# stone-d-chen/ffvvc

Measured on AMD Instinct MI355X. Metric: decoded frames/sec (4K/8K 10-bit VVC) per GPU, higher is better.
Workload: dtype u16

## Files before the change

### ffvvc_amd/csrc/loopfilter.hip

```cpp
#include "common.hpp"
#include "runtime.hpp"
#include "bs_rules.hpp"
#include "../../include/vvc_mi355.h"
#include "stage_checks.hpp"

namespace vvc355 {


template <int BD>
__global__ __launch_bounds__(256) void lmcs_kernel(const vvc355_blend_job *__restrict__ jobs)
{
    using px_t = typename Px<BD>::type;
    constexpr int VB = 8 * (int)sizeof(px_t);
    __shared__ __attribute__((aligned(16))) px_t lut_lds[1 << BD];
    const vvc355_blend_job job = load_uniform(jobs + (blockIdx.y));
    const uint8_t *lut = (const uint8_t *)job.src0;
    if ((job.src0 & 15) == 0) {
        for (int i = threadIdx.x; i < (int)((sizeof(px_t) << BD) / 16); i += 256)
            ((uint4 *)lut_lds)[i] = gld<uint4>(lut + i * 16);
    } else {
        for (int i = threadIdx.x; i < (1 << BD); i += 256)
            lut_lds[i] = (px_t)ld_px<BD>(lut, i);
    }
    __syncthreads();
// ... 430 lines not shown
    __device__ __forceinline__ void vec(int o, int n, int (&e)[4]) const
    {
        const px_t *a = (const px_t *)pix + o;
        if (BD > 8) {
            uint2 v = make_uint2(0, 0);
            if (n == 4) v = gld<uint2>(a); else v.x = gld<uint32_t>(a);
            e[0] = v.x & 0xffff; e[1] = v.x >> 16; e[2] = v.y & 0xffff; e[3] = v.y >> 16;
        } else {
            const uint32_t v = n == 4 ? gld<uint32_t>(a) : (uint32_t)gld<uint16_t>(a);
            e[0] = v & 0xff; e[1] = (v >> 8) & 0xff; e[2] = (v >> 16) & 0xff; e[3] = v >> 24;
        }
    }
    __device__ __forceinline__ void load(int lines, int half, int which)
    {
        const int b = 4 * half;
        if (xs == 1) {
#pragma unroll
            for (int l = 0; l < 4; l++) {
                int e[4];
                if (l < lines && (which & 1)) {
                    vec(l * ys - b - 4, 4, e);
#pragma unroll
                    for (int k = 0; k < 4; k++) P[l][b + 3 - k] = e[k];
                }
                if (l < lines && (which & 2)) {
                    vec(l * ys + b, 4, e);
#pragma unroll
                    for (int k = 0; k < 4; k++) Q[l][b + k] = e[k];
                }
            }
        } else {
#pragma unroll
            for (int i = 0; i < 4; i++) {
                int e[4];
                if (which & 1) {
                    vec(-(b + i + 1) * xs, lines, e);
#pragma unroll
                    for (int l = 0; l < 4; l++) P[l][b + i] = e[l];
                }
                if (which & 2) {
                    vec((b + i) * xs, lines, e);
#pragma unroll
                    for (int l = 0; l < 4; l++) Q[l][b + i] = e[l];
                }
            }
        }
    }
};
__device__ __forceinline__ int d2(int a, int b, int c) { return abs(a - 2 * b + c); }

__device__ __forceinline__ int long_w(int n, int i) { return n == 3 ? 53 - 21 * i : n == 5 ? 58 - 13 * i : 59 - 9 * i; }
__device__ __forceinline__ int long_t(int n, int i) { return n == 3 ? 6 - 2 * i : n == 5 ? 6 - i : max(6 - i, 1); }

template <int BD>
__device__ __forceinline__ void dbk_luma_large(const Dbk<BD> &d, int tc, int no_p, int no_q, int len_p, int len_q)
{
#pragma unroll
    for (int l = 0; l < 4; l++) {
        int p[8], q[8], m;
#pragma unroll
        for (int i = 0; i < 8; i++) { p[i] = d.p(l, i); q[i] = d.q(l, i); }
        if (len_p == 5 && len_q == 5)
            m = (p[4] + p[3] + 2 * (p[2] + p[1] + p[0] + q[0] + q[1] + q[2]) + q[3] + q[4] + 8) >> 4;
        else if (len_p == len_q)
            m = (p[6] + p[5] + p[4] + p[3] + p[2] + p[1] + 2 * (p[0] + q[0]) + q[1] + q[2] + q[3] + q[4] + q[5] + q[6] + 8) >> 4;
        else if (len_p + len_q == 12)
            m = (p[5] + p[4] + p[3] + p[2] + 2 * (p[1] + p[0] + q[0] + q[1]) + q[2] + q[3] + q[4] + q[5] + 8) >> 4;
        else if (len_p + len_q == 8)
            m = (p[3] + p[2] + p[1] + p[0] + q[0] + q[1] + q[2] + q[3] + 4) >> 3;
        else if (len_q == 7)
            m = (2 * (p[2] + p[1] + p[0] + q[0]) + p[0] + p[1] + q[1] + q[2] + q[3] + q[4] + q[5] + q[6] + 8) >> 4;
        else
            m = (p[6] + p[5] + p[4] + p[3] + p[2] + p[1] + 2 * (q[2] + q[1] + q[0] + p[0]) + q[0] + q[1] + 8) >> 4;
        if (!no_p) {
            const int n = len_p == 3 ? 3 : len_p == 5 ? 5 : 7;
            int ref = 0;
#pragma unroll
            for (int i = 0; i < 8; i++) if (i == len_p || i == len_p - 1) ref += p[i];
            ref = (ref + 1) >> 1;
#pragma unroll
            for (int i = 0; i < 7; i++)
                if (i < n) {
                    const int lim = (tc * long_t(n, i)) >> 1, wt = long_w(n, i);
                    d.sp(l, i, p[i] + clip3(((m * wt + ref * (64 - wt) + 32) >> 6) - p[i], -lim, lim));
                }
        }
        if (!no_q) {
            const int n = len_q == 3 ? 3 : len_q == 5 ? 5 : 7;
            int ref = 0;
#pragma unroll
            for (int i = 0; i < 8; i++) if (i == len_q || i == len_q - 1) ref += q[i];
            ref = (ref + 1) >> 1;
#pragma unroll
            for (int i = 0; i < 7; i++)
                if (i < n) {
                    const int lim = (tc * long_t(n, i)) >> 1, wt = long_w(n, i);
                    d.sq(l, i, q[i] + clip3(((m * wt + ref * (64 - wt) + 32) >> 6) - q[i], -lim, lim));
                }
        }
    }
}

template <int BD>
__device__ __forceinline__ void dbk_luma_segment(const Dbk<BD> &d, int tc_in, int beta_in, int no_p, int no_q, int len_p, int len_q, int hor_ctu_edge)
{
    const int tc = BD < 10 ? (tc_in + (1 << (9 - BD))) >> (10 - BD) : tc_in << (BD - 10);
    if (!tc)
        return;
    const int dp0 = d2(d.p(0, 2), d.p(0, 1), d.p(0, 0)), dq0 = d2(d.q(0, 2), d.q(0, 1), d.q(0, 0));
    const int dp3 = d2(d.p(3, 2), d.p(3, 1), d.p(3, 0)), dq3 = d2(d.q(3, 2), d.q(3, 1), d.q(3, 0));
    const int d0 = dp0 + dq0, d3 = dp3 + dq3;
    const int tc25 = (tc * 5 + 1) >> 1;
    const int large_p = len_p > 3 && !hor_ctu_edge, large_q = len_q > 3;
    const int beta = beta_in << (BD - 8);

    if (large_p || large_q) {
        const int dp0l = large_p ? (dp0 + d2(d.p(0, 5), d.p(0, 4), d.p(0, 3)) + 1) >> 1 : dp0;
        const int dq0l = large_q ? (dq0 + d2(d.q(0, 5), d.q(0, 4), d.q(0, 3)) + 1) >> 1 : dq0;
        const int dp3l = large_p ? (dp3 + d2(d.p(3, 5), d.p(3, 4), d.p(3, 3)) + 1) >> 1 : dp3;
        const int dq3l = large_q ? (dq3 + d2(d.q(3, 5), d.q(3, 4), d.q(3, 3)) + 1) >> 1 : dq3;
        const int d0l = dp0l + dq0l, d3l = dp3l + dq3l;
        const int beta53 = (beta * 3) >> 5, beta_4 = beta >> 4;
        len_p = large_p ? len_p : 3;
        len_q = large_q ? len_q : 3;
        if (d0l + d3l < beta) {
            const int sp0l = abs(d.p(0, 3) - d.p(0, 0)) + (len_p == 7 ? abs(d.p(0, 7) - d.p(0, 6) - d.p(0, 5) + d.p(0, 4)) : 0);
            const int sq0l = abs(d.q(0, 0) - d.q(0, 3)) + (len_q == 7 ? abs(d.q(0, 4) - d.q(0, 5) - d.q(0, 6) + d.q(0, 7)) : 0);
            const int sp3l = abs(d.p(3, 3) - d.p(3, 0)) + (len_p == 7 ? abs(d.p(3, 7) - d.p(3, 6) - d.p(3, 5) + d.p(3, 4)) : 0);
            const int sq3l = abs(d.q(3, 0) - d.q(3, 3)) + (len_q == 7 ? abs(d.q(3, 4) - d.q(3, 5) - d.q(3, 6) + d.q(3, 7)) : 0);
            const int sp0 = large_p ? (sp0l + abs(d.p(0, 3) - d.p_at(0, len_p)) + 1) >> 1 : sp0l;
            const int sp3 = large_p ? (sp3l + abs(d.p(3, 3) - d.p_at(3, len_p)) + 1) >> 1 : sp3l;
            const int sq0 = large_q ? (sq0l + abs(d.q(0, 3) - d.q_at(0, len_q)) + 1) >> 1 : sq0l;
            const int sq3 = large_q ? (sq3l + abs(d.q(3, 3) - d.q_at(3, len_q)) + 1) >> 1 : sq3l;
            if (sp0 + sq0 < beta53 && abs(d.p(0, 0) - d.q(0, 0)) < tc25 &&
                sp3 + sq3 < beta53 && abs(d.p(3, 0) - d.q(3, 0)) < tc25 &&
                (d0l << 1) < beta_4 && (d3l << 1) < beta_4) {
                dbk_luma_large<BD>(d, tc, no_p, no_q, len_p, len_q);
                return;
            }
        }
    }
    if (d0 + d3 >= beta)
        return;
    const int beta_3 = beta >> 3, beta_2 = beta >> 2;
    if (len_p > 2 && len_q > 2 &&
        abs(d.p(0, 3) - d.p(0, 0)) + abs(d.q(0, 3) - d.q(0, 0)) < beta_3 && abs(d.p(0, 0) - d.q(0, 0)) < tc25 &&
        abs(d.p(3, 3) - d.p(3, 0)) + abs(d.q(3, 3) - d.q(3, 0)) < beta_3 && abs(d.p(3, 0) - d.q(3, 0)) < tc25 &&
        (d0 << 1) < beta_2 && (d3 << 1) < beta_2) {
        const int tc2 = tc << 1, tc3 = tc * 3;
#pragma unroll
        for (int l = 0; l < 4; l++) {
            const int p3 = d.p(l, 3), p2 = d.p(l, 2), p1 = d.p(l, 1), p0 = d.p(l, 0);
            const int q0 = d.q(l, 0), q1 = d.q(l, 1), q2 = d.q(l, 2), q3 = d.q(l, 3);
            if (!no_p) {
                d.sp(l, 0, p0 + clip3(((p2 + 2 * p1 + 2 * p0 + 2 * q0 + q1 + 4) >> 3) - p0, -tc3, tc3));
                d.sp(l, 1, p1 + clip3(((p2 + p1 + p0 + q0 + 2) >> 2) - p1, -tc2, tc2));
                d.sp(l, 2, p2 + clip3(((2 * p3 + 3 * p2 + p1 + p0 + q0 + 4) >> 3) - p2, -tc, tc));
            }
            if (!no_q) {
                d.sq(l, 0, q0 + clip3(((p1 + 2 * p0 + 2 * q0 + 2 * q1 + q2 + 4) >> 3) - q0, -tc3, tc3));
                d.sq(l, 1, q1 + clip3(((p0 + q0 + q1 + q2 + 2) >> 2) - q1, -tc2, tc2));
                d.sq(l, 2, q2 + clip3(((2 * q3 + 3 * q2 + q1 + q0 + p0 + 4) >> 3) - q2, -tc, tc));
            }
        }
    } else {
        int nd_p = 1, nd_q = 1;
        if (len_p > 1 && len_q > 1) {
            const int side = (beta + (beta >> 1)) >> 3;
            if (dp0 + dp3 < side) nd_p = 2;
            if (dq0 + dq3 < side) nd_q = 2;
        }
        const int tc_2 = tc >> 1;
#pragma unroll
        for (int l = 0; l < 4; l++) {
            const int p2 = d.p(l, 2), p1 = d.p(l, 1), p0 = d.p(l, 0);
            const int q0 = d.q(l, 0), q1 = d.q(l, 1), q2 = d.q(l, 2);
            int delta = (9 * (q0 - p0) - 3 * (q1 - p1) + 8) >> 4;
            if (abs(delta) >= 10 * tc)
                continue;
            delta = clip3(delta, -tc, tc);
            if (!no_p) d.sp(l, 0, clip_px<BD>(p0 + delta));
            if (!no_q) d.sq(l, 0, clip_px<BD>(q0 - delta));
            if (!no_p && nd_p > 1) d.sp(l, 1, clip_px<BD>(p1 + clip3((((p2 + p0 + 1) >> 1) - p1 + delta) >> 1, -tc_2, tc_2)));
            if (!no_q && nd_q > 1) d.sq(l, 1, clip_px<BD>(q1 + clip3((((q2 + q0 + 1) >> 1) - q1 - delta) >> 1, -tc_2, tc_2)));
        }
    }
}

template <int BD>
__device__ __forceinline__ void dbk_chroma_segment(const Dbk<BD> &d, int lines, int tc_in, int beta_in, int no_p, int no_q, int len_p, int len_q)
{
    const int tc = BD < 10 ? (tc_in + (1 << (9 - BD))) >> (10 - BD) : tc_in << (BD - 10);
    if (!tc || !len_p || !len_q)
        return;
    const int l2 = lines == 2 ? 1 : 3;
    const int beta = beta_in << (BD - 8), beta_3 = beta >> 3, beta_2 = beta >> 2, tc25 = (tc * 5 + 1) >> 1;
    if (len_q == 3) {
        const bool one = len_p == 1;
        const int p0 = d.p(0, 0), p1 = d.p(0, 1), p2 = one ? p1 : d.p(0, 2), p3 = one ? p1 : d.p(0, 3);
        const int p0n = d.pn(l2, 0), p1n = d.pn(l2, 1), p2n = one ? p1n : d.pn(l2, 2);
        const int q0 = d.q(0, 0), q1 = d.q(0, 1), q2 = d.q(0, 2), q3 = d.q(0, 3);
        const int q0n = d.qn(l2, 0), q1n = d.qn(l2, 1), q2n = d.qn(l2, 2);
        const int dd0 = d2(p2, p1, p0) + d2(q2, q1, q0), dd1 = d2(p2n, p1n, p0n) + d2(q2n, q1n, q0n);
        bool strong = false;
        if (dd0 + dd1 < beta) {
            const int p3n = one ? p1n : d.pn(l2, 3), q3n = d.qn(l2, 3);
            const bool ok0 = (dd0 << 1) < beta_2 && abs(p3 - p0) + abs(q0 - q3) < beta_3 && abs(p0 - q0) < tc25;
            const bool ok1 = (dd1 << 1) < beta_2 && abs(p3n - p0n) + abs(q0n - q3n) < beta_3 && abs(p0n - q0n) < tc25;
            strong = ok0 && ok1;
        }
        if (!strong)
            len_p = len_q = 1;
    }
    const int kind = (len_p == 3 && len_q == 3) ? 2 : (len_q == 3) ? 1 : 0;
#pragma unroll
    for (int l = 0; l < 4; l++) {
        if (l >= lines)
            continue;
        const int p3 = d.p(l, 3), p2 = d.p(l, 2), p1 = d.p(l, 1), p0 = d.p(l, 0);
        const int q0 = d.q(l, 0), q1 = d.q(l, 1), q2 = d.q(l, 2), q3 = d.q(l, 3);
        if (kind == 2) {
            if (!no_p) {
                d.sp(l, 0, clip3((p3 + p2 + p1 + 2 * p0 + q0 + q1 + q2 + 4) >> 3, p0 - tc, p0 + tc));
                d.sp(l, 1, clip3((2 * p3 + p2 + 2 * p1 + p0 + q0 + q1 + 4) >> 3, p1 - tc, p1 + tc));
                d.sp(l, 2, clip3((3 * p3 + 2 * p2 + p1 + p0 + q0 + 4) >> 3, p2 - tc, p2 + tc));
            }
            if (!no_q) {
                d.sq(l, 0, clip3((p2 + p1 + p0 + 2 * q0 + q1 + q2 + q3 + 4) >> 3, q0 - tc, q0 + tc));
                d.sq(l, 1, clip3((p1 + p0 + q0 + 2 * q1 + q2 + 2 * q3 + 4) >> 3, q1 - tc, q1 + tc));
                d.sq(l, 2, clip3((p0 + q0 + q1 + 2 * q2 + 3 * q3 + 4) >> 3, q2 - tc, q2 + tc));
            }
        } else if (kind == 1) {
            if (!no_p)
                d.sp(l, 0, clip3((3 * p1 + 2 * p0 + q0 + q1 + q2 + 4) >> 3, p0 - tc, p0 + tc));
            if (!no_q) {
                d.sq(l, 0, clip3((2 * p1 + p0 + 2 * q0 + q1 + q2 + q3 + 4) >> 3, q0 - tc, q0 + tc));
                d.sq(l, 1, clip3((p1 + p0 + q0 + 2 * q1 + q2 + 2 * q3 + 4) >> 3, q1 - tc, q1 + tc));
                d.sq(l, 2, clip3((p0 + q0 + q1 + 2 * q2 + 3 * q3 + 4) >> 3, q2 - tc, q2 + tc));
            }
        } else {
            const int delta = clip3((((q0 - p0) * 4) + p1 - q1 + 4) >> 3, -tc, tc);
            if (!no_p) d.sp(l, 0, clip_px<BD>(p0 + delta));
            if (!no_q) d.sq(l, 0, clip_px<BD>(q0 - delta));
        }
    }
}

template <int BD>
__device__ __forceinline__ void deblock_luma_seg(uint8_t *pix, int xs, int ys, int tc, int beta, int no_p, int no_q, int len_p, int len_q, int flag)
{
    Dbk<BD> d;
    d.xs = xs; d.ys = ys; d.pix = pix;
    const int far = (len_p > 3 && !flag ? 1 : 0) | (len_q > 3 ? 2 : 0);
    d.load(4, 0, 3);
#pragma unroll
    for (int l = 0; l < 4; l++)
#pragma unroll
        for (int i = 4; i < 8; i++) d.P[l][i] = d.Q[l][i] = 0;
    if (far)
        d.load(4, 1, far);
    dbk_luma_segment<BD>(d, tc, beta, no_p, no_q, len_p, len_q, flag);
}
template <int BD>
__device__ __forceinline__ void deblock_chroma_seg(uint8_t *pix, int xs, int ys, int lines, int tc, int beta, int no_p, int no_q, int len_p, int len_q)
{
    Dbk<BD> d;
    d.xs = xs; d.ys = ys; d.pix = pix;
#pragma unroll
    for (int l = 0; l < 4; l++)
#pragma unroll
        for (int i = 0; i < 8; i++) d.P[l][i] = d.Q[l][i] = 0;
    d.load(lines, 0, 3);
    dbk_chroma_segment<BD>(d, lines, tc, beta, no_p, no_q, len_p, len_q);
}

template <int BD>
__global__ __launch_bounds__(256) void deblock_kernel(const vvc355_deblock_job *__restrict__ jobs, int n_jobs)
{
    const int t = blockIdx.x * blockDim.x + threadIdx.x;
    const int j = t >> 1;
    if (j >= n_jobs)
        return;
    const vvc355_deblock_job *jp = jobs + j;
    const uint32_t kind = gld<uint32_t>(&jp->dir);
    const int dir = kind & 0xff, chroma = (kind >> 8) & 0xff, flag = (kind >> 16) & 0xff;
    const int lines = chroma ? (flag ? 2 : 4) : 4;
    const int pxstride = gld<int32_t>(&jp->stride) / (int)sizeof(typename Px<BD>::type);
    uint8_t *pix0 = (uint8_t *)gld<uint64_t>(&jp->pix);
    const int xs = dir == 0 ? pxstride : 1, ys = dir == 0 ? 1 : pxstride;
    const int seg0 = t & 1;
    const int pxb = (int)sizeof(typename Px<BD>::type);
    if (!chroma) {
        deblock_luma_seg<BD>(pix0 + (ptrdiff_t)(seg0 * 4 * ys * pxb), xs, ys, gld<int32_t>(&jp->tc[seg0]), gld<int32_t>(&jp->beta[seg0]),
                             gld<uint8_t>(&jp->no_p[seg0]), gld<uint8_t>(&jp->no_q[seg0]), gld<uint8_t>(&jp->max_len_p[seg0]),
                             gld<uint8_t>(&jp->max_len_q[seg0]), flag);
        return;
    }
    for (int seg = seg0; seg < 8 / lines; seg += 2)
        deblock_chroma_seg<BD>(pix0 + (ptrdiff_t)(seg * lines * ys * pxb), xs, ys, lines, gld<int32_t>(&jp->tc[seg]), gld<int32_t>(&jp->beta[seg]),
                               gld<uint8_t>(&jp->no_p[seg]), gld<uint8_t>(&jp->no_q[seg]), gld<uint8_t>(&jp->max_len_p[seg]),
                               gld<uint8_t>(&jp->max_len_q[seg]));
}

#define VVC355_TABLE(type, name, count) __device__ static const type lf_tab_##name[count]
#include "tables_small.inc"
#undef VVC355_TABLE
#define kTcTable lf_tab_tc_table
#define kBetaTable lf_tab_beta_table

template <int BD>
__global__ __launch_bounds__(256) void deblock_frame_kernel(const vvc355_deblock_frame *__restrict__ fp, int u1, int u2, int n_units,
                                                            int na0, int na1, int ne0, int ne1)
{
    using px_t = typename Px<BD>::type;
    const vvc355_deblock_frame F = load_uniform(fp);
    const int vertical = F.vertical;
    __shared__ uint32_t slot[256];
    __shared__ int wave_cnt[4];
    uint32_t desc = 0;
    bool active = false;
    {
        const int t = blockIdx.x * blockDim.x + threadIdx.x;
        const int unit = t >> 1;
        if (unit < n_units) {
            if (unit >= u1) {
                active = true;
                desc = 0x80000000u | threadIdx.x;
            } else {
                const int n_edges = ne0, n_along = na0;
                int ke, ku;
                if (vertical) { ku = unit / n_edges; ke = unit - ku * n_edges; }
                else          { ke = unit / n_along; ku = unit - ke * n_along; }
                const int e = (ke + 1) * 4, u = ku * 8, seg = t & 1;
                const int x = vertical ? e : u + 4 * seg, y = vertical ? u + 4 * seg : e;
                if (vertical ? y < F.height : x < F.width) {
                    const int bs = gld<uint8_t>((const uint8_t *)F.bs[0] + (y >> 2) * F.min_tu_width + (x >> 2));
                    active = bs != 0;
                    desc = (uint32_t)x | ((uint32_t)y << 14) | ((uint32_t)bs << 28);
                }
            }
        }
    }
    const int wave = threadIdx.x >> 6, lane = threadIdx.x & 63;
    const uint64_t m = __ballot(active);
    if (lane == 0)
        wave_cnt[wave] = __popcll(m);
    __syncthreads();
    int base = 0, total = 0;
#pragma unroll
    for (int k = 0; k < 4; k++) {
        const int n = wave_cnt[k];
        if (k < wave) base += n;
        total += n;
    }
    if (active)
        slot[base + __popcll(m & ((1ull << lane) - 1))] = desc;
    __syncthreads();
    if ((int)threadIdx.x >= total)
        return;
    const uint32_t mine = slot[threadIdx.x];
    const bool is_chroma = mine >> 31;
    const int t = blockIdx.x * blockDim.x + (is_chroma ? (int)(mine & 255) : 0);
    const int unit = t >> 1;
    const int c = !is_chroma ? 0 : unit >= u2 ? 2 : 1;
    const int local = unit - (c == 2 ? u2 : c == 1 ? u1 : 0);
    const int n_along = c ? na1 : na0;
    const int hs = c ? F.hs : 0, vs = c ? F.vs : 0;
    const int grid = c ? (8 << (vertical ? hs : vs)) : 4, step = 8 << (vertical ? vs : hs);
    const int n_edges = c ? ne1 : ne0;
    int e, u;
    if (is_chroma) {
        int ke, ku;
        if (vertical) { ku = local / n_edges; ke = local - ku * n_edges; }
        else          { ke = local / n_along; ku = local - ke * n_along; }
        e = (ke + 1) * grid; u = ku * step;
    } else {
        const int x = mine & 0x3fff, y = (mine >> 14) & 0x3fff;
        e = vertical ? x : y; u = vertical ? y : x;
    }
    const int ux = vertical ? e : u, uy = vertical ? u : e;
    const int hor_ctu_edge = !vertical && !(e & ((1 << F.ctb_log2) - 1));
    const int ctb = (ux >> F.ctb_log2) + (uy >> F.ctb_log2) * F.ctb_width;
    const int8_t *dbp = (const int8_t *)F.db_params + ctb * 6;
    const int shift = vertical ? vs : hs, lines = c ? (shift ? 2 : 4) : 4, nseg = 8 / lines;
    const uint8_t *bs_tab = (const uint8_t *)sel3(c, F.bs);
    uint8_t *plane = (uint8_t *)sel3(c, F.plane);
    const int stride = sel3(c, F.stride), pxstride = stride / (int)sizeof(px_t);
    const int xs = vertical ? 1 : pxstride, ys = vertical ? pxstride : 1;
    if (!c) {
        const int x = mine & 0x3fff, y = (mine >> 14) & 0x3fff, bs = (mine >> 28) & 3;
        const int tu = (y >> 2) * F.min_tu_width + (x >> 2);
        const int xp = x - vertical, yp = y - !vertical;
        uint8_t *pix = plane + row_off(y, stride) + x * (int)sizeof(px_t);
        const int8_t *qy = (const int8_t *)F.qp_y;
        const int a = gld<int8_t>(qy + (xp >> F.min_cb_log2) + (yp >> F.min_cb_log2) * F.min_cb_width);
        const int b = gld<int8_t>(qy + (x >> F.min_cb_log2) + (y >> F.min_cb_log2) * F.min_cb_width);
        const int len_p = gld<uint8_t>((const uint8_t *)F.max_len_p + tu), len_q = gld<uint8_t>((const uint8_t *)F.max_len_q + tu);
        const int beta_offset = gld<int8_t>(dbp), tc_offset = gld<int8_t>(dbp + 3);
        int qp = (a + b + 1) >> 1;
        if (F.ladf_enabled) {
            const int level = (ld_px<BD>(pix, -xs) + ld_px<BD>(pix, -xs + 3 * ys) + ld_px<BD>(pix, 0) + ld_px<BD>(pix, 3 * ys)) >> 2;
            int qp_offset = F.ladf_lowest_qp_offset;
            bool go = true;
#pragma unroll
            for (int k = 0; k < 4; k++) {
                go = go && k < F.num_ladf_intervals - 1 && level > F.ladf_lower_bound[k + 1];
                if (go)
                    qp_offset = F.ladf_qp_offset[k];
            }
            qp += qp_offset;
        }
        const int beta = gld<uint8_t>(kBetaTable + clip3(qp + beta_offset, 0, 63));
        const int tc = gld<uint16_t>(kTcTable + clip3(qp + 2 * (bs - 1) + (tc_offset & -2), 0, 65));
        deblock_luma_seg<BD>(pix, xs, ys, tc, beta, 0, 0, len_p, len_q, hor_ctu_edge);
        return;
    }
    const int8_t *qc = (const int8_t *)(c == 1 ? F.qp_c[0] : F.qp_c[1]);
    const uint8_t *tbs = (const uint8_t *)F.tb_size_c;
    for (int seg = t & 1; seg < nseg; seg += 2) {
        const int x = vertical ? e : u + 4 * seg, y = vertical ? u + 4 * seg : e;
        if (vertical ? y >= F.height : x >= F.width)
            continue;
        const int tu = (y >> 2) * F.min_tu_width + (x >> 2);
        const int bs = gld<uint8_t>(bs_tab + tu);
        if (!bs)
            continue;
        const int xp = x - vertical, yp = y - !vertical;
        const int tup = (yp >> 2) * F.min_tu_width + (xp >> 2);
        uint8_t *pix = plane + row_off(y >> vs, stride) + (x >> hs) * (int)sizeof(px_t);
        const int qp = (gld<int8_t>(qc + tup) + gld<int8_t>(qc + tu) - 2 * F.qp_bd_offset + 1) >> 1;
        const int size_p = gld<uint8_t>(tbs + tup), size_q = gld<uint8_t>(tbs + tu);
        int len_p, len_q;
        if (size_p >= 8 && size_q >= 8) {
            len_q = 3;
            len_p = hor_ctu_edge ? 1 : 3;
        } else {
            len_p = len_q = bs == 2;
        }
        const int beta_offset = gld<int8_t>(dbp + c), tc_offset = gld<int8_t>(dbp + 3 + c);
        const int beta = gld<uint8_t>(kBetaTable + clip3(qp + beta_offset, 0, 63));
        const int tc = gld<uint16_t>(kTcTable + clip3(qp + 2 * (bs - 1) + (tc_offset & -2), 0, 65));
        deblock_chroma_seg<BD>(pix, xs, ys, lines, tc, beta, 0, 0, len_p, len_q);
    }
}

template <int BD>
__global__ void ladf_kernel(const uint8_t *pix, ptrdiff_t xs, ptrdiff_t ys, int *out)
{
    *out = (ld_px<BD>(pix, -xs) + ld_px<BD>(pix, -xs + 3 * ys) + ld_px<BD>(pix, 0) + ld_px<BD>(pix, 3 * ys)) >> 2;
}


static void launch_sao(int bd, const vvc355_sao_job *jobs, int n, int max_w, int max_h, hipStream_t st)
{
    if (n <= 0) return;
    const int gx = max(1, min(16, (max_w * max_h + 1023) / 1024));
    VVC355_BD_DISPATCH(bd, hipLaunchKernelGGL((sao_kernel<BD>), dim3(gx, n), dim3(256), 0, st, jobs));
    HIP_CHECK(hipGetLastError());
}

static void launch_sao_vec(int bd, const vvc355_sao_job *jobs, int n, int max_h, hipStream_t st)
{
    if (n <= 0) return;
    VVC355_BD_DISPATCH(bd, hipLaunchKernelGGL((sao_vec_kernel<BD>), dim3((max_h + 63) / 64, n), dim3(256), 0, st, jobs));
    HIP_CHECK(hipGetLastError());
}

static void launch_deblock(int bd, const vvc355_deblock_job *jobs, int n, hipStream_t st)
{
    if (n <= 0) return;
    VVC355_BD_DISPATCH(bd, hipLaunchKernelGGL((deblock_kernel<BD>), dim3((n * 2 + 255) / 256), dim3(256), 0, st, jobs, n));
    HIP_CHECK(hipGetLastError());
}

static void slot_deblock(int bd, int dir, int chroma, uint8_t *pix, ptrdiff_t stride, const int32_t *beta, const int32_t *tc,
                         const uint8_t *no_p, const uint8_t *no_q, const uint8_t *max_len_p, const uint8_t *max_len_q, int flag)
{
    const int px = bd > 8 ? 2 : 1;
    const int nseg = chroma ? (flag ? 4 : 2) : 2;
    SlotCall call;
    const Staged s = dir == 0 ? call.rect(pix, stride, 0, 8 * px, -8, 8, true, true)
                              : call.rect(pix, stride, -8 * px, 8 * px, 0, 8, true, true);
    vvc355_deblock_job job = {};
    job.pix = (uint64_t)s.dev; job.stride = (int32_t)s.pitch;
    job.dir = (uint8_t)dir; job.chroma = (uint8_t)chroma; job.flag = (uint8_t)flag;
    for (int i = 0; i < nseg; i++) {
        job.beta[i] = beta[i]; job.tc[i] = tc[i];
        job.no_p[i] = no_p[i]; job.no_q[i] = no_q[i]; job.max_len_p[i] = max_len_p[i]; job.max_len_q[i] = max_len_q[i];
    }
    launch_deblock(bd, call.upload(&job, 1), 1, call.stream());
}


__global__ __launch_bounds__(256) void deblock_bs_kernel(const vvc355_bs_frame *__restrict__ fp)
{
    const vvc355_bs_frame F = load_uniform(fp);
    const int mtw = F.min_tu_width, mpw = F.min_pu_width, mcl = F.min_cb_log2, mcw = F.min_cb_width;
    const int ux = blockIdx.x * 64 + (threadIdx.x & 63), uy = blockIdx.y * 4 + (threadIdx.x >> 6);
    const int x = ux * 4, y = uy * 4;
    if (x >= F.width || y >= F.height)
        return;
    const int off = uy * mtw + ux;
    const int ctb_log2 = F.ctb_log2, ctb_mask = (1 << ctb_log2) - 1;
    const vvc355_mvfield *mvf = (const vvc355_mvfield *)F.mvf;
    const int16_t *slice = (const int16_t *)F.slice_idx;
    const int ctb = (y >> ctb_log2) * F.ctb_width + (x >> ctb_log2);

    const int has_n[2] = { uy > 0, ux > 0 };
    const int offn[2] = { has_n[0] ? off - mtw : off, has_n[1] ? off - 1 : off };
    const vvc355_mvfield curr = ld_mvf(mvf + uy * mpw + ux);
    const vvc355_mvfield neigh[2] = { ld_mvf(mvf + (uy - has_n[0]) * mpw + ux), ld_mvf(mvf + uy * mpw + ux - has_n[1]) };
    int t0[2][2];
#pragma unroll
    for (int t = 0; t < 2; t++) {
        t0[t][1] = gld<int>((const int *)F.tb_pos_x0[t] + off);
        t0[t][0] = gld<int>((const int *)F.tb_pos_y0[t] + off);
    }
    const int size_q[2] = { gld<uint8_t>((const uint8_t *)F.tb_height[0] + off), gld<uint8_t>((const uint8_t *)F.tb_width[0] + off) };
    const int size_p[2] = { gld<uint8_t>((const uint8_t *)F.tb_height[0] + offn[0]), gld<uint8_t>((const uint8_t *)F.tb_width[0] + offn[1]) };
    const uint8_t *flag_tab[6] = { (const uint8_t *)F.pcmf[0], (const uint8_t *)F.tu_coded_flag[0], (const uint8_t *)F.pcmf[1],
                                   (const uint8_t *)F.tu_coded_flag[1], (const uint8_t *)F.tu_coded_flag[2], (const uint8_t *)F.tu_joint_cbcr };
    int fq[6], fn[2][6];
#pragma unroll
    for (int k = 0; k < 6; k++) {
        fq[k] = gld<uint8_t>(flag_tab[k] + off);
        fn[0][k] = gld<uint8_t>(flag_tab[k] + offn[0]);
        fn[1][k] = gld<uint8_t>(flag_tab[k] + offn[1]);
    }
    int sb_p[2];
#pragma unroll
    for (int d = 0; d < 2; d++) {
        const int px = d ? x - has_n[1] : x, py = d ? y : y - has_n[0];
        const int cbp = (py >> mcl) * mcw + (px >> mcl);
        sb_p[d] = gld<uint8_t>((const uint8_t *)F.msf + cbp) | gld<uint8_t>((const uint8_t *)F.iaf + cbp);
    }
    const int my_slice = gld<int16_t>(slice + ctb);
    int n_slice[2], tile_edge[2];
#pragma unroll
    for (int d = 0; d < 2; d++) {
        const int a = d ? x : y;
        const bool on_ctb_edge = a > 0 && !(a & ctb_mask);
        n_slice[d] = gld<int16_t>(slice + (on_ctb_edge ? (d ? ctb - 1 : ctb - F.ctb_width) : ctb));
        const int16_t *bd = (const int16_t *)(d ? F.ctb_to_col_bd : F.ctb_to_row_bd);
        const int r = max(a >> ctb_log2, 1);
        tile_edge[d] = on_ctb_edge && gld<int16_t>(bd + r) != gld<int16_t>(bd + r - 1);
    }
    const int tx0 = t0[0][1], ty0 = t0[0][0];
    const bool is_intra = gld<uint8_t>((const uint8_t *)(mvf + (ty0 >> 2) * mpw + (tx0 >> 2)) + 20) == 0;
    const int cbo = (ty0 >> mcl) * mcw + (tx0 >> mcl);
    const int cb0[2] = { gld<int>((const int *)F.cb_pos_y + cbo), gld<int>((const int *)F.cb_pos_x + cbo) };
    const int cb_size[2] = { gld<uint8_t>((const uint8_t *)F.cb_height + cbo), gld<uint8_t>((const uint8_t *)F.cb_width + cbo) };
    const bool sb_cu = !is_intra && (gld<uint8_t>((const uint8_t *)F.msf + cbo) | gld<uint8_t>((const uint8_t *)F.iaf + cbo));

#define BS_RULES_OUT(tab, v) gst<uint8_t>((uint8_t *)(tab) + off, (uint8_t)(v))
#include "bs_rules_body.inc"
#undef BS_RULES_OUT
}

}

int vvc355::lmcs_frame_check(const vvc355_lmcs_frame *f, int bd)
{
    if (!f)
        return VVC355_LMCS_FRAME_E_FRAME;
    if (bd != 8 && bd != 10 && bd != 12)
        return VVC355_LMCS_FRAME_E_BD;
    if (f->width <= 0 || f->height <= 0 || f->width >= (1 << 16) || f->height >= (1 << 16))
        return VVC355_LMCS_FRAME_E_SIZE;
    if (f->ctb_log2 < 5 || f->ctb_log2 > 7)
        return VVC355_LMCS_FRAME_E_CTB;
    const int ctb = 1 << f->ctb_log2;
    if (f->ctb_width != (f->width + ctb - 1) >> f->ctb_log2 || f->ctb_height != (f->height + ctb - 1) >> f->ctb_log2)
        return VVC355_LMCS_FRAME_E_GRID;
    const int px = bd > 8 ? 2 : 1;
    if (f->stride < f->width * px || f->stride % px || f->stride >= (1 << 23) || (int64_t)f->stride * f->height >= ((int64_t)1 << 31))
        return VVC355_LMCS_FRAME_E_STRIDE;
    if (f->n_slices < 0)
        return VVC355_LMCS_FRAME_E_COUNT;
    if (!f->plane || !f->inv_lut || !f->slice_idx || !f->slice_lmcs_used)
        return VVC355_LMCS_FRAME_E_TABLES;
    return 0;
}

using namespace vvc355;

extern "C" {

void vvc355_sao_batch(void *stream, int bd, const vvc355_sao_job *jobs_dev, int n_jobs, int max_w, int max_h)
{
    if (n_jobs <= 0) return;
    launch_sao(bd, jobs_dev, n_jobs, max_w, max_h, (hipStream_t)stream);
}

void vvc355_deblock_bs_pass(void *stream, const vvc355_bs_frame *frame_dev, const vvc355_bs_frame *frame_host)
{
    const vvc355_bs_frame &F = *frame_host;
    if (F.width <= 0 || F.height <= 0) return;
    if ((F.width & 3) || (F.height & 3) || F.min_tu_width < F.width / 4 || F.min_pu_width < F.width / 4) {
        fprintf(stderr, "vvc_mi355: deblock_bs_pass: %dx%d with table pitches %d / %d outside the driver's domain\n", F.width, F.height, F.min_tu_width, F.min_pu_width);
        abort();
    }
    const int nx = F.width / 4, ny = F.height / 4;
    hipLaunchKernelGGL(deblock_bs_kernel, dim3((nx + 63) / 64, (ny + 3) / 4), dim3(256), 0, (hipStream_t)stream, frame_dev);
    HIP_CHECK(hipGetLastError());
}

void vvc355_sao_frame_pass(void *stream, int bd, const vvc355_sao_frame *frame_dev, const vvc355_sao_frame *frame_host)
{
    const vvc355_sao_frame &F = *frame_host;
    const int n = F.ctb_width * F.ctb_height;
    if (n <= 0) return;
    const int ctb = 1 << F.ctb_log2;
    auto rows_per_wg = [](int w) { const int lxl = w > 64 ? 4 : w > 32 ? 3 : w > 16 ? 2 : w > 8 ? 1 : 0; return (256 >> lxl) * 4; };
    const int tiles_l = (ctb + rows_per_wg(ctb) - 1) / rows_per_wg(ctb);
    int tiles_c = 0, packed = 0;
    if (F.n_comp >= 3) {
        const int wc = ctb >> F.hs, hc = ctb >> F.vs;
        packed = 2 * hc <= rows_per_wg(wc);
        tiles_c = (hc + rows_per_wg(wc) - 1) / rows_per_wg(wc);
    }
    const int gx = tiles_l + (F.n_comp >= 3 ? (packed ? 1 : 2 * tiles_c) : 0);
    VVC355_BD_DISPATCH(bd, hipLaunchKernelGGL((sao_frame_kernel<BD>), dim3(gx, n), dim3(256), 0, (hipStream_t)stream, frame_dev, 4 * gx,
                                              tiles_l, tiles_c, packed));
    HIP_CHECK(hipGetLastError());
}

void vvc355_sao_ctb_batch(void *stream, int bd, const vvc355_sao_job *jobs_dev, int n_jobs, int max_h)
{
    if (n_jobs <= 0) return;
    launch_sao_vec(bd, jobs_dev, n_jobs, max_h, (hipStream_t)stream);
}

void vvc355_deblock_frame_pass(void *stream, int bd, const vvc355_deblock_frame *frame_dev, const vvc355_deblock_frame *frame_host)
{
    if (frame_host->width >= (1 << 14) || frame_host->height >= (1 << 14)) {
        fprintf(stderr, "vvc_mi355: deblock_frame_pass: picture %dx%d beyond the 14-bit segment coordinates\n", frame_host->width, frame_host->height);
        abort();
    }
    const vvc355_deblock_frame &F = *frame_host;
    int first[4] = { 0, 0, 0, 0 }, n_along[2] = { 0, 0 }, n_edge[2] = { 0, 0 };
    for (int c = 0; c < F.n_comp; c++) {
        const int hs = c ? F.hs : 0, vs = c ? F.vs : 0;
        const int grid = c ? (8 << (F.vertical ? hs : vs)) : 4, step = 8 << (F.vertical ? vs : hs);
        const int across = F.vertical ? F.width : F.height, along = F.vertical ? F.height : F.width;
        const int n_edges = (across - 1) / grid, n_units = (along + step - 1) / step;
        n_along[c ? 1 : 0] = n_units;
        n_edge[c ? 1 : 0] = n_edges;
        first[c + 1] = first[c] + n_edges * n_units;
    }
    const int total = first[F.n_comp];
    if (total <= 0) return;
    VVC355_BD_DISPATCH(bd, hipLaunchKernelGGL((deblock_frame_kernel<BD>), dim3((total * 2 + 255) / 256), dim3(256), 0, (hipStream_t)stream,
                                              frame_dev, first[1], F.n_comp > 2 ? first[2] : total, total, n_along[0], n_along[1], n_edge[0], n_edge[1]));
    HIP_CHECK(hipGetLastError());
}

void vvc355_deblock_batch(void *stream, int bd, const vvc355_deblock_job *jobs_dev, int n_jobs)
{
    if (n_jobs <= 0) return;
    launch_deblock(bd, jobs_dev, n_jobs, (hipStream_t)stream);
}

void vvc355_lmcs_batch(void *stream, int bd, const vvc355_blend_job *jobs_dev, int n_jobs, int max_w, int max_h)
{
    if (n_jobs <= 0) return;
    const int gx = max(1, min(64, (max_w * max_h + 8191) / 8192));
    VVC355_BD_DISPATCH(bd, hipLaunchKernelGGL((lmcs_kernel<BD>), dim3(gx, n_jobs), dim3(256), 0, (hipStream_t)stream, jobs_dev));
    HIP_CHECK(hipGetLastError());
}

int vvc355_lmcs_frame_pass(void *stream, int bd, const vvc355_lmcs_frame *frame_dev, const vvc355_lmcs_frame *frame_host)
{
    const int err = frame_dev ? lmcs_frame_check(frame_host, bd) : VVC355_LMCS_FRAME_E_FRAME;
    if (err)
        return err;
    const int ctb = 1 << frame_host->ctb_log2;
    const int gy = max(1, ctb * ctb / 8192);
    VVC355_BD_DISPATCH(bd, hipLaunchKernelGGL((lmcs_frame_kernel<BD>), dim3(frame_host->ctb_width * frame_host->ctb_height, gy), dim3(256), 0,
                                              (hipStream_t)stream, frame_dev));
    HIP_CHECK(hipGetLastError());
    return 0;
}

void vvc355_lmcs_filter(int bd, uint8_t *dst, ptrdiff_t dst_stride, int width, int height, const uint8_t *lut)
{
    if (width <= 0 || height <= 0) return;
    const int px = bd > 8 ? 2 : 1;
    SlotCall call;
    const Staged d = call.rect(dst, dst_stride, 0, width * px, 0, height, true, true);
    vvc355_blend_job job = {};
    job.dst = (uint64_t)d.dev; job.dst_stride = (int32_t)d.pitch;
    job.src0 = (uint64_t)call.linear(lut, (size_t)px << bd, true, false);
    job.w = (int16_t)width; job.h = (int16_t)height;
    vvc355_lmcs_batch(call.stream(), bd, call.upload(&job, 1), 1, width, height);
}

void vvc355_sao_band_filter(int bd, uint8_t *dst, const uint8_t *src, ptrdiff_t dst_stride, ptrdiff_t src_stride,
                            const int16_t *sao_offset_val, int sao_left_class, int width, int height)
{
    if (width <= 0 || height <= 0) return;
    const int px = bd > 8 ? 2 : 1;
    SlotCall call;
    const Staged s = call.rect(src, src_stride, 0, width * px, 0, height, true, false);
    const Staged d = call.rect(dst, dst_stride, 0, width * px, 0, height, false, true);
    vvc355_sao_job job = {};
    job.dst = (uint64_t)d.dev; job.src = (uint64_t)s.dev; job.dst_stride = (int32_t)d.pitch; job.src_stride = (int32_t)s.pitch;
    job.w = (int16_t)width; job.h = (int16_t)height; job.type = 1; job.band_position = (uint8_t)sao_left_class;
    for (int k = 0; k < 5; k++) job.offset_val[k] = sao_offset_val[k];
    launch_sao(bd, call.upload(&job, 1), 1, width, height, call.stream());
}

void vvc355_sao_edge_filter(int bd, uint8_t *dst, const uint8_t *src, ptrdiff_t dst_stride,
                            const int16_t *sao_offset_val, int eo, int width, int height)
{
    if (width <= 0 || height <= 0) return;
    const int px = bd > 8 ? 2 : 1;
    const ptrdiff_t src_stride = 2 * VVC355_PB + 64;
    SlotCall call;
    const Staged s = call.rect(src, src_stride, -px, (width + 1) * px, -1, height + 1, true, false);
    const Staged d = call.rect(dst, dst_stride, 0, width * px, 0, height, false, true);
    vvc355_sao_job job = {};
    job.dst = (uint64_t)d.dev; job.src = (uint64_t)s.dev; job.dst_stride = (int32_t)d.pitch; job.src_stride = (int32_t)s.pitch;
    job.w = (int16_t)width; job.h = (int16_t)height; job.type = 2; job.eo = (uint8_t)eo;
    for (int k = 0; k < 5; k++) job.offset_val[k] = sao_offset_val[k];
    launch_sao(bd, call.upload(&job, 1), 1, width, height, call.stream());
}

void vvc355_sao_edge_restore(int bd, int variant, uint8_t *dst, const uint8_t *src, ptrdiff_t dst_stride, ptrdiff_t src_stride,
                             const int16_t *offset_val, int eo_class, const int *borders, int width, int height,
                             const uint8_t *vert_edge, const uint8_t *horiz_edge, const uint8_t *diag_edge)
{
    if (width <= 0 || height <= 0) return;
    const int px = bd > 8 ? 2 : 1;
    SlotCall call;
    const Staged s = call.rect(src, src_stride, 0, width * px, 0, height, true, false);
    const Staged d = call.rect(dst, dst_stride, 0, width * px, 0, height, true, true);
    vvc355_sao_job job = {};
    job.dst = (uint64_t)d.dev; job.src = (uint64_t)s.dev; job.dst_stride = (int32_t)d.pitch; job.src_stride = (int32_t)s.pitch;
    job.w = (int16_t)width; job.h = (int16_t)height; job.type = 4; job.eo = (uint8_t)eo_class; job.restore = (uint8_t)!!variant;
    for (int k = 0; k < 5; k++) job.offset_val[k] = offset_val[k];
    for (int k = 0; k < 4; k++) { job.borders[k] = (uint8_t)!!borders[k]; job.diag_edge[k] = variant ? diag_edge[k] : 0; }
    for (int k = 0; k < 2; k++) { job.vert_edge[k] = variant ? vert_edge[k] : 0; job.horiz_edge[k] = variant ? horiz_edge[k] : 0; }
    launch_sao(bd, call.upload(&job, 1), 1, width, height, call.stream());
}

// ... 31 lines not shown
```

Baseline: 601.2.

## Deblock with packed 16-bit SIMD filters and vectorized register-tile loads

New measurement: 609.3, median of 6. 1.4% higher.

```diff
diff --git a/ffvvc_amd/csrc/loopfilter.hip b/ffvvc_amd/csrc/loopfilter.hip
--- a/ffvvc_amd/csrc/loopfilter.hip
+++ b/ffvvc_amd/csrc/loopfilter.hip
@@ -756,6 +756,316 @@
                                gld<uint8_t>(&jp->max_len_q[seg]));
 }
 
+typedef unsigned short upk16 __attribute__((ext_vector_type(2)));
+__device__ __forceinline__ upk16 upk(pk16 v) { return __builtin_bit_cast(upk16, v); }
+__device__ __forceinline__ upk16 upk_splat(int v) { return upk16{ (unsigned short)v, (unsigned short)v }; }
+__device__ __forceinline__ pk16 pk_abs(pk16 v) { return pk_max(v, pk_splat(0) - v); }
+__device__ __forceinline__ pk16 pk_clip(pk16 v, pk16 lo, pk16 hi) { return pk_max(pk_min(v, hi), lo); }
+__device__ __forceinline__ pk16 pk_clip_sym(pk16 v, int lim) { return pk_clip(v, pk_splat(-lim), pk_splat(lim)); }
+__device__ __forceinline__ pk16 pk_sel(bool c, pk16 a, pk16 b) { return pk(c ? un(a) : un(b)); }
+__device__ __forceinline__ pk16 pk_d2(pk16 a, pk16 b, pk16 c) { return pk_abs(a - b - b + c); }
+__device__ __forceinline__ pk16 pk_sar(pk16 v, int n) { return v >> pk_splat(n); }
+__device__ __forceinline__ uint32_t opaque(uint32_t v) { asm("" : "+v"(v)); return v; }
+__device__ __forceinline__ int pk_lo(pk16 v) { return v.x; }
+__device__ __forceinline__ int pk_hi(pk16 v) { return v.y; }
+
+template <int BD> struct DbkPk {
+    using px_t = typename Px<BD>::type;
+    uint8_t *pix;
+    int xs, ys, lines;
+    bool vert;
+    uint32_t P[8][2], Q[8][2];
+
+    __device__ __forceinline__ pk16 dec(const uint32_t (&r)[2]) const
+    {
+        return pk(lines == 2 ? r[0] : __builtin_amdgcn_perm(r[1], r[0], 0x07060100u));
+    }
+    __device__ __forceinline__ void row(int o, uint32_t (&r)[2]) const
+    {
+        const px_t *a = (const px_t *)pix + o;
+        if (BD > 8) {
+            if (lines == 4) { const uint2 v = gld<uint2>(a); r[0] = v.x; r[1] = v.y; }
+            else { r[0] = gld<uint32_t>(a); r[1] = 0; }
+        } else {
+            const uint32_t v = lines == 4 ? gld<uint32_t>(a) : (uint32_t)gld<uint16_t>(a);
+            r[0] = __builtin_amdgcn_perm(0, v, 0x0c010c00u); r[1] = __builtin_amdgcn_perm(0, v, 0x0c030c02u);
+        }
+    }
+    __device__ __forceinline__ void load(int half, int which)
+    {
+        const int b = 4 * half;
+        if (vert) {
+#pragma unroll
+            for (int s = 0; s < 2; s++) {
+                if (!(which & (1 << s)))
+                    continue;
+                uint32_t L[4][2];
+#pragma unroll
+                for (int l = 0; l < 4; l++) {
+                    L[l][0] = L[l][1] = 0;
+                    if (l < lines) {
+                        const px_t *a = (const px_t *)pix + l * ys + (s ? b : -b - 4);
+                        if (BD > 8) { const uint2 v = gld<uint2>(a); L[l][0] = v.x; L[l][1] = v.y; }
+                        else L[l][0] = gld<uint32_t>(a);
+                    }
+                }
+#pragma unroll
+                for (int k = 0; k < 4; k++)
+#pragma unroll
+                    for (int j = 0; j < 2; j++) {
+                        const uint32_t t = BD > 8 ? __builtin_amdgcn_perm(L[2 * j + 1][k >> 1], L[2 * j][k >> 1], (k & 1) ? 0x07060302u : 0x05040100u)
+                                                  : __builtin_amdgcn_perm(L[2 * j + 1][0], L[2 * j][0], 0x0c040c00u + k * 0x00010001u);
+                        if (s) Q[b + k][j] = t; else P[b + 3 - k][j] = t;
+                    }
+            }
+        } else {
+#pragma unroll
+            for (int i = 0; i < 4; i++) {
+                if (which & 1) row(-(b + i + 1) * xs, P[b + i]);
+                if (which & 2) row((b + i) * xs, Q[b + i]);
+            }
+        }
+    }
+    __device__ __forceinline__ void put_row(int o, const uint32_t (&r)[2]) const
+    {
+        px_t *a = (px_t *)pix + o;
+        if (BD > 8) {
+            if (lines == 4) gst<uint2>(a, make_uint2(r[0], r[1])); else gst<uint32_t>(a, r[0]);
+        } else {
+            const uint32_t v = __builtin_amdgcn_perm(r[1], r[0], 0x06040200u);
+            if (lines == 4) gst<uint32_t>(a, v); else gst<uint16_t>(a, (uint16_t)v);
+        }
+    }
+    __device__ __forceinline__ void put_pair(int o, uint32_t first, uint32_t second, int h) const
+    {
+        px_t *a = (px_t *)pix + o;
+        if (BD > 8) gst<uint32_t>(a, __builtin_amdgcn_perm(second, first, h ? 0x07060302u : 0x05040100u));
+        else gst<uint16_t>(a, (uint16_t)__builtin_amdgcn_perm(second, first, h ? 0x0c0c0602u : 0x0c0c0400u));
+    }
+    __device__ __forceinline__ void store(int np, int nq) const
+    {
+        if (!vert) {
+#pragma unroll
+            for (int i = 0; i < 7; i++) {
+                if (i < np) put_row(-(i + 1) * xs, P[i]);
+                if (i < nq) put_row(i * xs, Q[i]);
+            }
+            return;
+        }
+#pragma unroll
+        for (int l = 0; l < 4; l++) {
+            if (l >= lines)
+                continue;
+            const int j = l >> 1, h = l & 1;
+#pragma unroll
+            for (int i = 0; i < 7; i += 2) {
+                if (i + 1 < 7 && i + 1 < np) put_pair(l * ys - i - 2, P[i + 1][j], P[i][j], h);
+                else if (i < np) st_px<BD>(pix, l * ys - i - 1, h ? P[i][j] >> 16 : P[i][j] & 0xffff);
+                if (i + 1 < 7 && i + 1 < nq) put_pair(l * ys + i, Q[i][j], Q[i + 1][j], h);
+                else if (i < nq) st_px<BD>(pix, l * ys + i, h ? Q[i][j] >> 16 : Q[i][j] & 0xffff);
+            }
+        }
+    }
+};
+
+#define PJ(i) pk(d.P[i][j])
+#define QJ(i) pk(d.Q[i][j])
+
+template <int BD>
+__device__ __forceinline__ void dbk_luma_large_pk(DbkPk<BD> &d, int tc, int len_p, int len_q, int &np, int &nq)
+{
+    static_assert(BD <= 10, "the packed filters keep their intermediates in 16 bits: see the ranges above");
+#define MID(expr, sh) do { _Pragma("unroll") for (int j = 0; j < 2; j++) m[j] = pk_sar((expr) + pk_splat(1 << ((sh) - 1)), sh); } while (0)
+    pk16 m[2];
+    if (len_p == 5 && len_q == 5)
+        MID(PJ(4) + PJ(3) + (PJ(2) + PJ(1) + PJ(0) + QJ(0) + QJ(1) + QJ(2)) * pk_splat(2) + QJ(3) + QJ(4), 4);
+    else if (len_p == len_q)
+        MID(PJ(6) + PJ(5) + PJ(4) + PJ(3) + PJ(2) + PJ(1) + (PJ(0) + QJ(0)) * pk_splat(2) + QJ(1) + QJ(2) + QJ(3) + QJ(4) + QJ(5) + QJ(6), 4);
+    else if (len_p + len_q == 12)
+        MID(PJ(5) + PJ(4) + PJ(3) + PJ(2) + (PJ(1) + PJ(0) + QJ(0) + QJ(1)) * pk_splat(2) + QJ(2) + QJ(3) + QJ(4) + QJ(5), 4);
+    else if (len_p + len_q == 8)
+        MID(PJ(3) + PJ(2) + PJ(1) + PJ(0) + QJ(0) + QJ(1) + QJ(2) + QJ(3), 3);
+    else if (len_q == 7)
+        MID((PJ(2) + PJ(1) + PJ(0) + QJ(0)) * pk_splat(2) + PJ(0) + PJ(1) + QJ(1) + QJ(2) + QJ(3) + QJ(4) + QJ(5) + QJ(6), 4);
+    else
+        MID(PJ(6) + PJ(5) + PJ(4) + PJ(3) + PJ(2) + PJ(1) + (QJ(2) + QJ(1) + QJ(0) + PJ(0)) * pk_splat(2) + QJ(0) + QJ(1), 4);
+    np = len_p == 3 ? 3 : len_p == 5 ? 5 : 7;
+    nq = len_q == 3 ? 3 : len_q == 5 ? 5 : 7;
+    pk16 ref_p[2], ref_q[2];
+#pragma unroll
+    for (int j = 0; j < 2; j++) {
+        const uint32_t p32 = opaque(un(PJ(3) + PJ(2))), p54 = opaque(un(PJ(5) + PJ(4))), p76 = opaque(un(PJ(7) + PJ(6)));
+        const uint32_t q32 = opaque(un(QJ(3) + QJ(2))), q54 = opaque(un(QJ(5) + QJ(4))), q76 = opaque(un(QJ(7) + QJ(6)));
+        const uint32_t sp = len_p == 3 ? p32 : len_p == 5 ? p54 : p76;
+        const uint32_t sq = len_q == 3 ? q32 : len_q == 5 ? q54 : q76;
+        ref_p[j] = pk_sar(pk(sp) + pk_splat(1), 1);
+        ref_q[j] = pk_sar(pk(sq) + pk_splat(1), 1);
+    }
+#pragma unroll
+    for (int i = 0; i < 7; i++) {
+        if (i < np) {
+            const int lim = (tc * long_t(np, i)) >> 1, wt = long_w(np, i);
+#pragma unroll
+            for (int j = 0; j < 2; j++) {
+                const upk16 v = (upk(m[j]) * upk_splat(wt) + upk(ref_p[j]) * upk_splat(64 - wt) + upk_splat(32)) >> upk_splat(6);
+                d.P[i][j] = un(PJ(i) + pk_clip_sym(__builtin_bit_cast(pk16, v) - PJ(i), lim));
+            }
+        }
+        if (i < nq) {
+            const int lim = (tc * long_t(nq, i)) >> 1, wt = long_w(nq, i);
+#pragma unroll
+            for (int j = 0; j < 2; j++) {
+                const upk16 v = (upk(m[j]) * upk_splat(wt) + upk(ref_q[j]) * upk_splat(64 - wt) + upk_splat(32)) >> upk_splat(6);
+                d.Q[i][j] = un(QJ(i) + pk_clip_sym(__builtin_bit_cast(pk16, v) - QJ(i), lim));
+            }
+        }
+    }
+#undef MID
+}
+
+template <int BD>
+__device__ __forceinline__ void dbk_luma_segment_pk(DbkPk<BD> &d, int tc_in, int beta_in, int len_p, int len_q, int hor_ctu_edge, int &np, int &nq)
+{
+    static_assert(BD <= 10, "the packed filters keep their intermediates in 16 bits: see the ranges above");
+    np = nq = 0;
+    const int tc = BD < 10 ? (tc_in + (1 << (9 - BD))) >> (10 - BD) : tc_in << (BD - 10);
+    if (!tc)
+        return;
+    const pk16 p0 = d.dec(d.P[0]), p1 = d.dec(d.P[1]), p2 = d.dec(d.P[2]), p3 = d.dec(d.P[3]);
+    const pk16 q0 = d.dec(d.Q[0]), q1 = d.dec(d.Q[1]), q2 = d.dec(d.Q[2]), q3 = d.dec(d.Q[3]);
+    const pk16 dp = pk_d2(p2, p1, p0), dq = pk_d2(q2, q1, q0), dd = dp + dq;
+    const pk16 apq = pk_abs(p0 - q0);
+    const int tc25 = (tc * 5 + 1) >> 1;
+    const int large_p = len_p > 3 && !hor_ctu_edge, large_q = len_q > 3;
+    const int beta = beta_in << (BD - 8);
+
+    if (large_p || large_q) {
+        const pk16 p4 = d.dec(d.P[4]), p5 = d.dec(d.P[5]), p6 = d.dec(d.P[6]), p7 = d.dec(d.P[7]);
+        const pk16 q4 = d.dec(d.Q[4]), q5 = d.dec(d.Q[5]), q6 = d.dec(d.Q[6]), q7 = d.dec(d.Q[7]);
+        const pk16 dpl = pk_sel(large_p, pk_sar(dp + pk_d2(p5, p4, p3) + pk_splat(1), 1), dp);
+        const pk16 dql = pk_sel(large_q, pk_sar(dq + pk_d2(q5, q4, q3) + pk_splat(1), 1), dq);
+        const pk16 ddl = dpl + dql;
+        const int beta53 = (beta * 3) >> 5, beta_4 = beta >> 4;
+        len_p = large_p ? len_p : 3;
+        len_q = large_q ? len_q : 3;
+        if (pk_lo(ddl) + pk_hi(ddl) < beta) {
+            const pk16 spl = pk_abs(p3 - p0) + pk_sel(len_p == 7, pk_abs(p7 - p6 - p5 + p4), pk_splat(0));
+            const pk16 sql = pk_abs(q0 - q3) + pk_sel(len_q == 7, pk_abs(q4 - q5 - q6 + q7), pk_splat(0));
+            const pk16 p_at = pk_sel(len_p == 7, p7, pk_sel(len_p == 5, p5, p3)), q_at = pk_sel(len_q == 7, q7, pk_sel(len_q == 5, q5, q3));
+            const pk16 sp = pk_sel(large_p, pk_sar(spl + pk_abs(p3 - p_at) + pk_splat(1), 1), spl);
+            const pk16 sq = pk_sel(large_q, pk_sar(sql + pk_abs(q3 - q_at) + pk_splat(1), 1), sql);
+            const pk16 s = sp + sq;
+            if (pk_lo(s) < beta53 && pk_lo(apq) < tc25 && pk_hi(s) < beta53 && pk_hi(apq) < tc25 &&
+                (pk_lo(ddl) << 1) < beta_4 && (pk_hi(ddl) << 1) < beta_4) {
+                dbk_luma_large_pk<BD>(d, tc, len_p, len_q, np, nq);
+                return;
+            }
+        }
+    }
+    if (pk_lo(dd) + pk_hi(dd) >= beta)
+        return;
+    const int beta_3 = beta >> 3, beta_2 = beta >> 2;
+    const pk16 s3 = pk_abs(p3 - p0) + pk_abs(q3 - q0);
+    if (len_p > 2 && len_q > 2 &&
+        pk_lo(s3) < beta_3 && pk_lo(apq) < tc25 && pk_hi(s3) < beta_3 && pk_hi(apq) < tc25 &&
+        (pk_lo(dd) << 1) < beta_2 && (pk_hi(dd) << 1) < beta_2) {
+        const int tc2 = tc << 1, tc3 = tc * 3;
+#pragma unroll
+        for (int j = 0; j < 2; j++) {
+            const pk16 P3 = PJ(3), P2 = PJ(2), P1 = PJ(1), P0 = PJ(0), Q0 = QJ(0), Q1 = QJ(1), Q2 = QJ(2), Q3 = QJ(3);
+            const pk16 mid = P0 + Q0, two = pk_splat(2), four = pk_splat(4);
+            d.P[0][j] = un(P0 + pk_clip_sym(pk_sar(P2 + (P1 + mid) * two + Q1 + four, 3) - P0, tc3));
+            d.P[1][j] = un(P1 + pk_clip_sym(pk_sar(P2 + P1 + mid + two, 2) - P1, tc2));
+            d.P[2][j] = un(P2 + pk_clip_sym(pk_sar(P3 * two + P2 * pk_splat(3) + P1 + mid + four, 3) - P2, tc));
+            d.Q[0][j] = un(Q0 + pk_clip_sym(pk_sar(P1 + (mid + Q1) * two + Q2 + four, 3) - Q0, tc3));
+            d.Q[1][j] = un(Q1 + pk_clip_sym(pk_sar(mid + Q1 + Q2 + two, 2) - Q1, tc2));
+            d.Q[2][j] = un(Q2 + pk_clip_sym(pk_sar(Q3 * two + Q2 * pk_splat(3) + Q1 + mid + four, 3) - Q2, tc));
+        }
+        np = nq = 3;
+    } else {
+        np = nq = 1;
+        if (len_p > 1 && len_q > 1) {
+            const int side = (beta + (beta >> 1)) >> 3;
+            if (pk_lo(dp) + pk_hi(dp) < side) np = 2;
+            if (pk_lo(dq) + pk_hi(dq) < side) nq = 2;
+        }
+        const int tc_2 = tc >> 1;
+        const pk16 zero = pk_splat(0), top = pk_splat((1 << BD) - 1), one = pk_splat(1);
+#pragma unroll
+        for (int j = 0; j < 2; j++) {
+            const pk16 P2 = PJ(2), P1 = PJ(1), P0 = PJ(0), Q0 = QJ(0), Q1 = QJ(1), Q2 = QJ(2);
+            const pk16 raw = pk_sar((Q0 - P0) * pk_splat(9) - (Q1 - P1) * pk_splat(3) + pk_splat(8), 4);
+            const uint32_t keep = un(pk_sar(pk_abs(raw) - pk_splat(10 * tc), 15));
+            const pk16 delta = pk_clip_sym(raw, tc);
+            const pk16 n_p0 = pk_clip(P0 + delta, zero, top), n_q0 = pk_clip(Q0 - delta, zero, top);
+            const pk16 n_p1 = pk_clip(P1 + pk_clip_sym(pk_sar(pk_sar(P2 + P0 + one, 1) - P1 + delta, 1), tc_2), zero, top);
+            const pk16 n_q1 = pk_clip(Q1 + pk_clip_sym(pk_sar(pk_sar(Q2 + Q0 + one, 1) - Q1 - delta, 1), tc_2), zero, top);
+            d.P[0][j] = (un(n_p0) & keep) | (d.P[0][j] & ~keep);
+            d.Q[0][j] = (un(n_q0) & keep) | (d.Q[0][j] & ~keep);
+            d.P[1][j] = (un(n_p1) & keep) | (d.P[1][j] & ~keep);
+            d.Q[1][j] = (un(n_q1) & keep) | (d.Q[1][j] & ~keep);
+        }
+    }
+}
+
+template <int BD>
+__device__ __forceinline__ void dbk_chroma_segment_pk(DbkPk<BD> &d, int tc_in, int beta_in, int len_p, int len_q, int &np, int &nq)
+{
+    static_assert(BD <= 10, "the packed filters keep their intermediates in 16 bits: see the ranges above");
+    np = nq = 0;
+    const int tc = BD < 10 ? (tc_in + (1 << (9 - BD))) >> (10 - BD) : tc_in << (BD - 10);
+    if (!tc || !len_p || !len_q)
+        return;
+    const int beta = beta_in << (BD - 8), beta_3 = beta >> 3, beta_2 = beta >> 2, tc25 = (tc * 5 + 1) >> 1;
+    if (len_q == 3) {
+        const bool one = len_p == 1;
+        const pk16 p0 = d.dec(d.P[0]), p1 = d.dec(d.P[1]), p2 = pk_sel(one, p1, d.dec(d.P[2])), p3 = pk_sel(one, p1, d.dec(d.P[3]));
+        const pk16 q0 = d.dec(d.Q[0]), q1 = d.dec(d.Q[1]), q2 = d.dec(d.Q[2]), q3 = d.dec(d.Q[3]);
+        const pk16 dd = pk_d2(p2, p1, p0) + pk_d2(q2, q1, q0);
+        bool strong = false;
+        if (pk_lo(dd) + pk_hi(dd) < beta) {
+            const pk16 s3 = pk_abs(p3 - p0) + pk_abs(q0 - q3), apq = pk_abs(p0 - q0);
+            strong = (pk_lo(dd) << 1) < beta_2 && pk_lo(s3) < beta_3 && pk_lo(apq) < tc25 &&
+                     (pk_hi(dd) << 1) < beta_2 && pk_hi(s3) < beta_3 && pk_hi(apq) < tc25;
+        }
+        if (!strong)
+            len_p = len_q = 1;
+    }
+    const int kind = (len_p == 3 && len_q == 3) ? 2 : (len_q == 3) ? 1 : 0;
+    const pk16 t = pk_splat(tc), two = pk_splat(2), three = pk_splat(3), four = pk_splat(4);
+#pragma unroll
+    for (int j = 0; j < 2; j++) {
+        if (2 * j >= d.lines)
+            continue;
+        const pk16 P3 = PJ(3), P2 = PJ(2), P1 = PJ(1), P0 = PJ(0), Q0 = QJ(0), Q1 = QJ(1), Q2 = QJ(2), Q3 = QJ(3);
+        if (kind == 2) {
+            d.P[0][j] = un(pk_clip(pk_sar(P3 + P2 + P1 + P0 * two + Q0 + Q1 + Q2 + four, 3), P0 - t, P0 + t));
+            d.P[1][j] = un(pk_clip(pk_sar(P3 * two + P2 + P1 * two + P0 + Q0 + Q1 + four, 3), P1 - t, P1 + t));
+            d.P[2][j] = un(pk_clip(pk_sar(P3 * three + P2 * two + P1 + P0 + Q0 + four, 3), P2 - t, P2 + t));
+        } else if (kind == 1) {
+            d.P[0][j] = un(pk_clip(pk_sar(P1 * three + P0 * two + Q0 + Q1 + Q2 + four, 3), P0 - t, P0 + t));
+        }
+        if (kind == 2) {
+            d.Q[0][j] = un(pk_clip(pk_sar(P2 + P1 + P0 + Q0 * two + Q1 + Q2 + Q3 + four, 3), Q0 - t, Q0 + t));
+        } else if (kind == 1) {
+            d.Q[0][j] = un(pk_clip(pk_sar(P1 * two + P0 + Q0 * two + Q1 + Q2 + Q3 + four, 3), Q0 - t, Q0 + t));
+        }
+        if (kind) {
+            d.Q[1][j] = un(pk_clip(pk_sar(P1 + P0 + Q0 + Q1 * two + Q2 + Q3 * two + four, 3), Q1 - t, Q1 + t));
+            d.Q[2][j] = un(pk_clip(pk_sar(P0 + Q0 + Q1 + Q2 * two + Q3 * three + four, 3), Q2 - t, Q2 + t));
+        } else {
+            const pk16 zero = pk_splat(0), top = pk_splat((1 << BD) - 1);
+            const pk16 delta = pk_clip_sym(pk_sar((Q0 - P0) * four + P1 - Q1 + four, 3), tc);
+            d.P[0][j] = un(pk_clip(P0 + delta, zero, top));
+            d.Q[0][j] = un(pk_clip(Q0 - delta, zero, top));
+        }
+    }
+    np = kind == 2 ? 3 : 1;
+    nq = kind ? 3 : 1;
+}
+#undef PJ
+#undef QJ
+
 #define VVC355_TABLE(type, name, count) __device__ static const type lf_tab_##name[count]
 #include "tables_small.inc"
 #undef VVC355_TABLE
@@ -852,8 +1162,24 @@
         const int len_p = gld<uint8_t>((const uint8_t *)F.max_len_p + tu), len_q = gld<uint8_t>((const uint8_t *)F.max_len_q + tu);
         const int beta_offset = gld<int8_t>(dbp), tc_offset = gld<int8_t>(dbp + 3);
         int qp = (a + b + 1) >> 1;
+        DbkPk<BD> dk;
+        if constexpr (BD <= 10) {
+            dk.pix = pix; dk.xs = xs; dk.ys = ys; dk.lines = 4; dk.vert = vertical;
+            dk.load(0, 3);
+#pragma unroll
+            for (int i = 4; i < 8; i++) dk.P[i][0] = dk.P[i][1] = dk.Q[i][0] = dk.Q[i][1] = 0;
+            const int far = (len_p > 3 && !hor_ctu_edge ? 1 : 0) | (len_q > 3 ? 2 : 0);
+            if (far)
+                dk.load(1, far);
+        }
         if (F.ladf_enabled) {
-            const int level = (ld_px<BD>(pix, -xs) + ld_px<BD>(pix, -xs + 3 * ys) + ld_px<BD>(pix, 0) + ld_px<BD>(pix, 3 * ys)) >> 2;
+            int level;
+            if constexpr (BD <= 10) {
+                const pk16 s = dk.dec(dk.P[0]) + dk.dec(dk.Q[0]);
+                level = (pk_lo(s) + pk_hi(s)) >> 2;
+            } else {
+                level = (ld_px<BD>(pix, -xs) + ld_px<BD>(pix, -xs + 3 * ys) + ld_px<BD>(pix, 0) + ld_px<BD>(pix, 3 * ys)) >> 2;
+            }
             int qp_offset = F.ladf_lowest_qp_offset;
             bool go = true;
 #pragma unroll
@@ -866,7 +1192,13 @@
         }
         const int beta = gld<uint8_t>(kBetaTable + clip3(qp + beta_offset, 0, 63));
         const int tc = gld<uint16_t>(kTcTable + clip3(qp + 2 * (bs - 1) + (tc_offset & -2), 0, 65));
-        deblock_luma_seg<BD>(pix, xs, ys, tc, beta, 0, 0, len_p, len_q, hor_ctu_edge);
+        if constexpr (BD <= 10) {
+            int np, nq;
+            dbk_luma_segment_pk<BD>(dk, tc, beta, len_p, len_q, hor_ctu_edge, np, nq);
+            dk.store(np, nq);
+        } else {
+            deblock_luma_seg<BD>(pix, xs, ys, tc, beta, 0, 0, len_p, len_q, hor_ctu_edge);
+        }
         return;
     }
     const int8_t *qc = (const int8_t *)(c == 1 ? F.qp_c[0] : F.qp_c[1]);
@@ -894,7 +1226,16 @@
         const int beta_offset = gld<int8_t>(dbp + c), tc_offset = gld<int8_t>(dbp + 3 + c);
         const int beta = gld<uint8_t>(kBetaTable + clip3(qp + beta_offset, 0, 63));
         const int tc = gld<uint16_t>(kTcTable + clip3(qp + 2 * (bs - 1) + (tc_offset & -2), 0, 65));
-        deblock_chroma_seg<BD>(pix, xs, ys, lines, tc, beta, 0, 0, len_p, len_q);
+        if constexpr (BD <= 10) {
+            DbkPk<BD> dk;
+            dk.pix = pix; dk.xs = xs; dk.ys = ys; dk.lines = lines; dk.vert = vertical;
+            dk.load(0, 3);
+            int np, nq;
+            dbk_chroma_segment_pk<BD>(dk, tc, beta, len_p, len_q, np, nq);
+            dk.store(np, nq);
+        } else {
+            deblock_chroma_seg<BD>(pix, xs, ys, lines, tc, beta, 0, 0, len_p, len_q);
+        }
     }
 }
 
```
